# boqian333/E2ENet-Medical

Measured on AMD Instinct MI355X. Metric: voxels/sec (train step fwd+bwd+update), 128^3 patch 32ch density=0.2, higher is better.
Workload: dtype f32 (fp16x2 split products, f32 accumulate); 1 GPU; BraTS-shaped 4-modal 128^3 patches, shiftConvPP base 32, K=4, DSFF density 0.2, batch 2 per GPU, fwd+loss+bwd+clip+SGD+mask step, dense (parity) wgrad; parallelism=dp1

## Files before the change

e2enet_medical_amd/_lib.py:

```python
import ctypes as C
import os

_HERE = os.path.dirname(os.path.abspath(__file__))
LIB_PATH = os.environ.get("E2E_LIB_PATH") or os.path.join(_HERE, "csrc", "libe2e_hip.so")

KNOWN_ENV = frozenset({
    "E2E_CONV_MM", "E2E_MM_GRID", "E2E_MM_GEOM", "E2E_MM_PAIRQ", "E2E_CONV_DENSE", "E2E_CONV_SPARSE2", "E2E_CONV_PERSIST", "E2E_CONV_WGS",
    "E2E_CONV_KSPLIT", "E2E_WG_H2", "E2E_WG_BF3", "E2E_CT_BF3", "E2E_CT_H2",
    "E2E_CONV_DBG", "E2E_MM_STAMPS",
    "E2E_LIB_PATH", "E2E_STRICT_ENV", "E2E_DENSE_MIN_DENSITY", "E2E_MM_MIN_DENSITY", "E2E_WGRAD_STREAM", "E2E_LANES", "E2E_GRAPHS",
    "E2E_GRAPH_MAX_VOXELS", "E2E_PLAN_CACHE_GB", "E2E_SW_BLOCKING", "E2E_FORCE_DIST",
    "E2E_CPU_THREADS", "E2E_BENCH_DRY", "E2E_BENCH_DRY_FAIL_RANK", "E2E_BENCH_ALL_LAUNCHES",
})


def check_env(environ=None, strict=None):
    environ = os.environ if environ is None else environ
    unknown = sorted(k for k in environ if k.startswith("E2E_") and k not in KNOWN_ENV)
    if not unknown:
        return
    msg = ("unknown E2E_* environment variable(s) %s: not read by this build (known: %s)"
           % (", ".join(unknown), ", ".join(sorted(KNOWN_ENV))))
    if strict is None:
        strict = environ.get("E2E_STRICT_ENV") == "1"
# ... 77 lines not shown
    "e2e_conv133_mm_ws_bytes": (LL, [I, I, I, I, I, I, I, I, I]),
    "e2e_conv133_mm_pack": (I, [P, I, LL, P]),
    "e2e_conv133_input_ranges_ws_bytes": (LL, [I]),
    "e2e_conv133_input_ranges": (I, [P, I, P, P]),
    "e2e_absmax_word": (I, [P, LL, P, P]),
    "e2e_conv133_fwd_mm": (I, [P, I, P, P, P, P, P, P, I, I, I, I, I, P]),
    "e2e_conv133_dgrad_mm": (I, [P, P, P, P, P, I, I, I, I, I, I, P]),
    "e2e_conv133_dgrad_dense": (I, [P, P, P, P, I, I, I, I, I, I, P, LL, P]),
    "e2e_conv133_wgrad_ws_bytes": (LL, [I, I, I, I, I, I, I, I, I]),
    "e2e_conv133_wgrad": (I, [P, P, P, P, I, I, I, I, I, I, I, I, I, P, P, P]),
    "e2e_diag_split_gemm": (I, [P, P, P, I, I, P, P]),
    "e2e_diag_kernel_clock": (I, [I, P, P, I]),
    "e2e_in_stats_finalize": (I, [P, I, P, P, F, P, P, P, P, I, I, P]),
    "e2e_in_lrelu_bwd_ws_doubles": (LL, [I, I]),
    "e2e_in_lrelu_bwd": (I, [P, P, P, P, P, P, P, F, P, P, P, P, I, I, LL, P, I, P, P]),
    "e2e_convT_fwd": (I, [P, P, P, F, P, P, P, I, I, I, I, I, I, I, I, I, P, P, P]),
    "e2e_convT_dgrad": (I, [P, P, P, P, I, I, I, I, I, I, I, I, I, I, P, P, P, P]),
    "e2e_convT_wgrad_ws_bytes": (LL, [I, I, I, I, I, I, I, I, I]),
    "e2e_convT_wgrad": (I, [P, P, P, F, P, P, P, I, I, I, I, I, I, I, I, I, P, P, P, P]),
    "e2e_maxpool_fwd": (I, [P, P, P, F, P, I, I, I, I, I, I, I, I, P]),
    "e2e_maxpool_bwd_num_records": (I, [I, I, I, I, I, I]),
    "e2e_maxpool_bwd": (I, [P, P, P, F, P, P, I, I, I, I, I, I, I, I, I, P, P, P, P]),
    "e2e_head1x1_fwd": (I, [P, P, P, F, P, P, I, I, I, LL, P]),
    "e2e_head1x1_dgrad": (I, [P, P, P, I, I, I, I, LL, P]),
    "e2e_head1x1_wgrad_ws_bytes": (LL, [I, I, I, LL]),
    "e2e_head1x1_wgrad": (I, [P, P, P, F, P, P, P, I, I, I, LL, P]),
    "e2e_loss_ws_bytes": (LL, [I, I]),
    "e2e_dc_ce_reduce": (I, [P, P, P, I, I, LL, P]),
    "e2e_dc_ce_grad": (I, [P, P, P, F, I, F, P, P, I, I, LL, P]),
    "e2e_dc_ce_fold_batch": (I, [P, I, I, P]),
    "e2e_online_eval_counts": (I, [P, P, P, I, I, LL, P]),
    "e2e_dc_bce_reduce": (I, [P, P, P, P, I, I, LL, P]),
    "e2e_dc_bce_grad": (I, [P, P, P, P, F, I, F, P, P, I, I, LL, P]),
    "e2e_online_eval_regions": (I, [P, P, P, P, I, I, LL, P]),
    "e2e_seg_to_regions": (I, [P, P, P, I, I, LL, P]),
    "e2e_ds_target_gather": (I, [P, P, P, P, P, I, I, I, I, I, I, I, P]),
    "e2e_grad_sqnorm": (I, [P, I, P, P]),
# ... 59 lines not shown
    "e2e_pp_select_ws_bytes": (LL, [LL, I]),
    "e2e_pp_select_count": (I, [P, LL, P, I, P, P, P]),
    "e2e_pp_select_coords": (I, [P, I, I, I, P, I, P, P, P, P, P, P]),
    "e2e_fingerprint_sample_chunk": (I, []),
    "e2e_fingerprint_sample_ws_bytes": (LL, [LL]),
    "e2e_fingerprint_sample_count": (I, [P, LL, P, P, P]),
    "e2e_fingerprint_sample_gather": (I, [P, P, I, LL, I, P, LL, P, P]),
    "e2e_fingerprint_stats_max_ranks": (I, []),
    "e2e_fingerprint_stats_ws_bytes": (LL, []),
    "e2e_fingerprint_stats": (I, [P, LL, P, I, P, P, P]),
    "e2e_loader_crop_max_batch": (I, []),
    "e2e_loader_crop": (I, [P, I, I, I, I, I, P, P, I, F, F, P]),
}

_NO_STATUS = {"e2e_last_error", "e2e_abi_version", "e2e_last_kernel", "e2e_conv133_num_partials", "e2e_conv133_wgrad_ws_bytes", "e2e_conv133_dense_ws_bytes", "e2e_conv133_mm_ws_bytes", "e2e_conv133_sparse_eligible", "e2e_conv133_sparse_wpk_floats", "e2e_maxpool_bwd_num_records", "e2e_conv133_fwd_ws_bytes", "e2e_conv133_dgrad_ws_bytes",
              "e2e_convT_wgrad_ws_bytes", "e2e_conv133_input_ranges_ws_bytes", "e2e_in_lrelu_bwd_ws_doubles", "e2e_head1x1_wgrad_ws_bytes", "e2e_loss_ws_bytes", "e2e_aug_stats_ws_bytes",
              "e2e_surface_max_line", "e2e_surface_distances_ws_bytes", "e2e_cc_ws_bytes", "e2e_pp_nonzero_ws_bytes", "e2e_pp_label_hist_bins",
              "e2e_pp_minmax_ws_bytes", "e2e_pp_norm_ws_bytes", "e2e_pp_select_chunk", "e2e_pp_select_max_classes", "e2e_pp_select_ws_bytes",
              "e2e_fingerprint_sample_chunk", "e2e_fingerprint_sample_ws_bytes", "e2e_fingerprint_stats_max_ranks",
              "e2e_fingerprint_stats_ws_bytes", "e2e_eval_census_max_slots", "e2e_eval_census_chunk", "e2e_eval_census_workgroups",
              "e2e_loader_crop_max_batch"}


class E2EError(RuntimeError):
    pass


class _Lib:
    def __init__(self, path):
        if not os.path.exists(path):
            raise ImportError(
# ... 12 lines not shown

    def _checked(self, name, fn):
        last_error = self._dll.e2e_last_error

        def call(*a):
            rc = fn(*a)
            if rc != 0:
                raise E2EError("%s failed (%d): %s" % (name, rc, (last_error() or b"").decode()))
        call.__name__ = name
        return call


_lib = None


ABI_VERSION = 24


def lib() -> _Lib:
    global _lib
    if _lib is None:
        import torch
        check_env()
        handle = _Lib(LIB_PATH)
        got = handle.abi_version()
        if got != ABI_VERSION:
            raise ImportError("%s reports ABI version %d, this package needs %d: rebuild with `make -C %s`"
                              % (LIB_PATH, got, ABI_VERSION, os.path.dirname(LIB_PATH)))
        _lib = handle
    return _lib
```

e2enet_medical_amd/csrc/api.hip:

```cpp
#include "e2e_common.h"
#include <cstring>

namespace e2e {
static thread_local char g_err[512] = "";
void set_error(const char* fmt, ...) {
  va_list ap;
  va_start(ap, fmt);
  vsnprintf(g_err, sizeof(g_err), fmt, ap);
  va_end(ap);
}
static thread_local char g_kernel[160] = "";
void note_kernel(const char* fmt, ...) {
  va_list ap;
  va_start(ap, fmt);
  vsnprintf(g_kernel, sizeof(g_kernel), fmt, ap);
  va_end(ap);
}
}

extern "C" const char* e2e_last_error(void) { return e2e::g_err; }
extern "C" const char* e2e_last_kernel(void) { return e2e::g_kernel; }
extern "C" int e2e_abi_version(void) { return 24; }

extern "C" int e2e_diag_kernel_clock(int family, double* mhz, double* busy_ms, int reset) {
  E2E_REQUIRE(mhz != nullptr && (family == 0 || family == 1), "diag_kernel_clock: family 0 (conv133_mm) or 1 (conv133_wgrad v5)");
  if (hipDeviceSynchronize() != hipSuccess) return e2e::check_launch("diag_kernel_clock");
  unsigned long long v[2] = {0, 0};
  if (family == 0) e2e::mm_clock_read(v, reset != 0); else e2e::wgrad_clock_read(v, reset != 0);
  *mhz = v[1] ? 100.0 * (double)v[0] / (double)v[1] : 0.0;
  if (busy_ms) *busy_ms = (double)v[1] / 1e5;
  return e2e::check_launch("diag_kernel_clock");
}
```

e2enet_medical_amd/csrc/e2e_common.h:

```cpp
#pragma once
#include <hip/hip_runtime.h>
#include <cstdio>
#include <cstdarg>
#include "e2e_hip.h"

typedef const float __attribute__((address_space(1)))* gfloat_p;

namespace e2e {

void set_error(const char* fmt, ...);
void note_kernel(const char* fmt, ...);

void mm_clock_read(unsigned long long out[2], bool reset);
void wgrad_clock_read(unsigned long long out[2], bool reset);

inline int check_launch(const char* what) {
  hipError_t e = hipGetLastError();
  if (e != hipSuccess) {
    set_error("%s: %s", what, hipGetErrorString(e));
    return E2E_ERR_LAUNCH;
  }
  return E2E_OK;
}

// ... 75 lines not shown
  const e2e_in_chan_t* chans;
  const float* dy;
  float* slab;
  int B, Cin, Cout, Di, Hi, Wi, Do, sd;
  int tiles_x, tiles_y, tiles_per_n, tiles_per_chunk;
  int segs;
  int cblocks;
  int geom;
  int h2;
  const unsigned* dy_absmax;
  const unsigned* x_absmax;
};
int launch_wgrad_bf3(const WgBf3Params& p, int nchunks, int pairs, hipStream_t st);
int reduce_slabs(const float* slab, float* dw, long long numel, int nslabs, hipStream_t st);

inline int split_tiles(long long total, int pairs, int target_wgs, int min_tiles, int* tiles_per_chunk) {
  long long want = target_wgs / (pairs > 0 ? pairs : 1);
  if (want < 1) want = 1;
  long long tpc = cdivll(total, want);
  if (tpc < min_tiles) tpc = min_tiles;
  if (tpc > total) tpc = total;
  *tiles_per_chunk = (int)tpc;
  return (int)cdivll(total, tpc);
}
inline int split_tiles_per_item(int tiles_per_n, int B, int pairs, int target_wgs, int min_tiles, int* tiles_per_chunk, int* segs) {
  long long want = target_wgs / (pairs > 0 ? pairs : 1);
  if (want < B) want = B;
  int tpc = cdiv(tiles_per_n, (int)(want / B));
  if (tpc < min_tiles) tpc = min_tiles;
  if (tpc > tiles_per_n) tpc = tiles_per_n;
// ... 7 lines not shown
```

e2enet_medical_amd/csrc/instnorm.hip:

```cpp
#include "e2e_common.h"
#include "e2e_split.h"

namespace {

struct Stat {
  double n, mean, m2;
};
__device__ __forceinline__ Stat combine(const Stat a, const Stat b) {
  if (b.n == 0.0) return a;
  if (a.n == 0.0) return b;
  Stat r;
  r.n = a.n + b.n;
  const double delta = b.mean - a.mean;
  r.mean = a.mean + delta * (b.n / r.n);
  r.m2 = a.m2 + b.m2 + delta * delta * (a.n * b.n / r.n);
  return r;
}

__global__ __launch_bounds__(256) void in_finalize_kernel(const double* __restrict__ part, int np,
                                                          const float* __restrict__ gamma,
                                                          const float* __restrict__ beta, float eps,
                                                          float* __restrict__ scale, float* __restrict__ shift,
                                                          float* __restrict__ mean_out, float* __restrict__ rstd_out,
                                                          int C) {
// ... 95 lines not shown
  __syncthreads();
  if (threadIdx.x == 0) {
    double* r = sums + ((long long)nc * gridDim.x + blockIdx.x) * 2;
    r[0] = sh[0][0] + sh[0][1] + sh[0][2] + sh[0][3];
    r[1] = sh[1][0] + sh[1][1] + sh[1][2] + sh[1][3];
  }
}

__global__ __launch_bounds__(256) void in_bwd_apply_kernel(float* __restrict__ dz, const float* __restrict__ y,
                                                           const float* __restrict__ mean,
                                                           const float* __restrict__ rstd,
                                                           const float* __restrict__ scale,
                                                           const float* __restrict__ shift,
                                                           const float* __restrict__ gamma, float slope,
                                                           double* __restrict__ sums, const double* __restrict__ rec, int nrec,
                                                           int B, int C, long long spatial, unsigned* __restrict__ absmax,
                                                           double* __restrict__ rec3) {
  const int nc = blockIdx.y;
  const int c = nc % C;
  const float mu = mean[nc], rs = rstd[nc], g = gamma[c], sca = scale[nc], shf = shift[nc];
  __shared__ double s12[2];
  if (rec != nullptr) {
    if (threadIdx.x < 64) {
      const double* r = rec + (long long)nc * nrec * 2;
      double a = 0.0, b = 0.0;
      for (int i = threadIdx.x; i < nrec; i += 64) { a += r[2 * i]; b += r[2 * i + 1]; }
      a = e2e::wave_sum_d(a);
      b = e2e::wave_sum_d(b);
      if (threadIdx.x == 0) {
        s12[0] = a; s12[1] = b;
        if (blockIdx.x == 0) { sums[(long long)nc * 3] = a; sums[(long long)nc * 3 + 1] = b; }
      }
    }
  } else if (threadIdx.x == 0) {
// ... 122 lines not shown

}

extern "C" int e2e_in_stats_finalize(const double* part, int np, const float* gamma, const float* beta, float eps,
                                     float* scale, float* shift, float* mean, float* rstd, int B, int C,
                                     void* stream) {
  E2E_REQUIRE(part && gamma && beta && scale && shift && mean && rstd, "in_stats_finalize: null pointer");
  E2E_REQUIRE(np > 0 && B > 0 && C > 0, "in_stats_finalize: bad dims");
  hipLaunchKernelGGL(in_finalize_kernel, dim3(B * C), dim3(256), 0, (hipStream_t)stream, part, np, gamma, beta, eps,
                     scale, shift, mean, rstd, C);
  return e2e::check_launch("in_finalize_kernel");
}

extern "C" long long e2e_in_lrelu_bwd_ws_doubles(int B, int C) { return (long long)B * C * (3 + 3 * 256) + 2; }

extern "C" int e2e_in_lrelu_bwd(float* dz_dy, const float* y, const float* mean, const float* rstd, const float* scale,
                                const float* shift, const float* gamma, float slope, float* dgamma, float* dbeta,
                                float* dbias, float* sums, int B, int C, long long spatial, const double* tile_sums, int np,
                                unsigned* dy_absmax, void* stream) {
  E2E_REQUIRE(dz_dy && y && mean && rstd && scale && shift && gamma && dgamma && dbeta && sums, "in_lrelu_bwd: null pointer");
  E2E_REQUIRE(B > 0 && C > 0 && spatial > 0, "in_lrelu_bwd: bad dims");
  hipStream_t st = (hipStream_t)stream;
  double* ds = reinterpret_cast<double*>(sums);
  double* recs = ds + (long long)B * C * 3;
  double* rec3 = recs + (long long)B * C * 256 * 2;
  long long blocks = e2e::cdivll(spatial, 256 * 4 * 4);
  if (blocks > 256) blocks = 256;
  if (blocks < 1) blocks = 1;
  dim3 grid((unsigned)blocks, B * C);
  if (tile_sums == nullptr) {
    hipLaunchKernelGGL(in_bwd_reduce_kernel, grid, dim3(256), 0, st, dz_dy, y, mean, rstd, scale, shift, slope, recs, C,
                       spatial, dy_absmax, ds);
    hipLaunchKernelGGL(in_bwd_apply_kernel, grid, dim3(256), 0, st, dz_dy, y, mean, rstd, scale, shift, gamma, slope, ds,
                       (const double*)recs, (int)blocks, B, C, spatial, dy_absmax, rec3);
  } else {
    E2E_REQUIRE(np > 0, "in_lrelu_bwd: tile_sums without a record count");
    hipLaunchKernelGGL(in_bwd_tile_sums_kernel, dim3(B * C), dim3(64), 0, st, tile_sums, ds, np, dy_absmax);
    hipLaunchKernelGGL(in_bwd_apply_kernel, grid, dim3(256), 0, st, dz_dy, y, mean, rstd, scale, shift, gamma, slope, ds,
                       (const double*)nullptr, 0, B, C, spatial, dy_absmax, rec3);
  }
  hipLaunchKernelGGL(in_bwd_params_kernel, dim3(C), dim3(64), 0, st, (const double*)ds, (const double*)rec3, (int)blocks,
                     dgamma, dbeta, dbias, B, C);
  return e2e::check_launch("in_lrelu_bwd");
}
```

e2enet_medical_amd/csrc/pool_head.hip:

```cpp
#include "e2e_common.h"

namespace {

__global__ __launch_bounds__(256) void maxpool_fwd_kernel(const float* __restrict__ x, const float* __restrict__ scale,
                                                          const float* __restrict__ shift, float slope,
                                                          float* __restrict__ y, int D, int H, int W, int kd, int kh, int kw,
                                                          int Do, int Ho, int Wo) {
  const int nc = blockIdx.y;
  const long long ospatial = (long long)Do * Ho * Wo;
  const long long oi = (long long)blockIdx.x * 256 + threadIdx.x;
  if (oi >= ospatial) return;
  const int wo = (int)(oi % Wo);
  const long long r = oi / Wo;
  const int ho = (int)(r % Ho), dq = (int)(r / Ho);
  float a = 1.f, b = 0.f, sl = 1.f;
  if (scale) { a = scale[nc]; b = shift[nc]; sl = slope; }
  const float* xp = x + (long long)nc * D * H * W;
  float m = -INFINITY;
  for (int i = 0; i < kd; ++i)
    for (int j = 0; j < kh; ++j)
      for (int k = 0; k < kw; ++k) {
        const float v = e2e::in_act(xp[((long long)(dq * kd + i) * H + (ho * kh + j)) * W + (wo * kw + k)], a, b, sl);
        m = (v > m || v != v) ? v : m;
      }
// ... 401 lines not shown
    hipLaunchKernelGGL(maxpool_fwd_w2_kernel, grid2, dim3(256), 0, (hipStream_t)stream, x, scale, shift, slope, y, D, H, W, kd,
                       kh, Do, Ho, Wo);
    return e2e::check_launch("maxpool_fwd_w2_kernel");
  }
  dim3 grid((unsigned)e2e::cdivll((long long)Do * Ho * Wo, 256), B * C);
  hipLaunchKernelGGL(maxpool_fwd_kernel, grid, dim3(256), 0, (hipStream_t)stream, x, scale, shift, slope, y, D, H, W, kd, kh,
                     kw, Do, Ho, Wo);
  return e2e::check_launch("maxpool_fwd_kernel");
}

extern "C" int e2e_maxpool_bwd_num_records(int D, int H, int W, int kd, int kh, int kw) {
  if (kd < 1 || kh < 1 || kd > 2 || kh > 2 || kw != 2 || (W % 4) != 0 || D % kd || H % kh) return 0;
  return (int)e2e::cdivll((long long)(D / kd) * (H / kh) * (W / 4), 256);
}

extern "C" int e2e_maxpool_bwd(const float* x, const float* scale, const float* shift, float slope, const float* dy,
                               float* dx, int accumulate, int B, int C, int D, int H, int W, int kd, int kh, int kw,
                               const float* mean, const float* rstd, double* tile_sums, void* stream) {
  E2E_REQUIRE(x && dy && dx, "maxpool_bwd: null pointer");
  E2E_REQUIRE(kd >= 1 && kh >= 1 && kw >= 1 && D >= kd && H >= kh && W >= kw, "maxpool_bwd: bad dims");
  E2E_REQUIRE(tile_sums == nullptr || (mean && rstd && scale && e2e_maxpool_bwd_num_records(D, H, W, kd, kh, kw) > 0),
              "maxpool_bwd: fused InstanceNorm-backward sums need a normalised source and a shape of e2e_maxpool_bwd_num_records");
  hipStream_t st = (hipStream_t)stream;
  const int Do = D / kd, Ho = H / kh, Wo = W / kw;
  if (!accumulate && (D % kd || H % kh || W % kw)) {
    e2e::zero_async(dx, (size_t)B * C * D * H * W * sizeof(float), st);
  }
  if (kw == 2 && (W % 4) == 0 && kd <= 2 && kh <= 2) {
    dim3 grid2((unsigned)e2e::cdivll((long long)Do * Ho * (Wo / 2), 256), B * C);
    hipLaunchKernelGGL(maxpool_bwd_w2_kernel, grid2, dim3(256), 0, st, x, scale, shift, slope, dy, dx, accumulate, D, H, W, kd, kh,
                       Do, Ho, Wo, mean, rstd, tile_sums);
    return e2e::check_launch("maxpool_bwd_w2_kernel");
  }
  dim3 grid((unsigned)e2e::cdivll((long long)Do * Ho * Wo, 256), B * C);
  hipLaunchKernelGGL(maxpool_bwd_kernel, grid, dim3(256), 0, st, x, scale, shift, slope, dy, dx, accumulate, D, H, W, kd, kh,
                     kw, Do, Ho, Wo);
  return e2e::check_launch("maxpool_bwd_kernel");
}

#define DISPATCH_KB(K, ...)                                   \
  if ((K) <= 4) { constexpr int KB = 4; __VA_ARGS__; }        \
  else if ((K) <= 8) { constexpr int KB = 8; __VA_ARGS__; }   \
  else { constexpr int KB = 16; __VA_ARGS__; }

extern "C" int e2e_head1x1_fwd(const float* x, const float* scale, const float* shift, float slope, const float* w,
                               float* logits, int B, int C, int K, long long spatial, void* stream) {
// ... 60 lines not shown
```

e2enet_medical_amd/engine.py:

```python
import contextlib
import ctypes as C
import math
import os
from typing import Dict, List, Optional, Sequence, Tuple

import torch

import numpy as np

from ._lib import lib, InChan, OutChan, ParamEntry, SparsePackJob, InSumChan, MmPackJob, RangeSrc, RangeJob

LRELU_SLOPE = 0.01
IN_EPS = 1e-5
DENSE_MIN_DENSITY = float(os.environ.get("E2E_DENSE_MIN_DENSITY", "0.5"))
WGRAD_STREAM = os.environ.get("E2E_WGRAD_STREAM", "1") != "0"
WGRAD_STREAM_MAX_ELEMS = 40000000
WGRAD_LATE = True
LANES = os.environ.get("E2E_LANES", "1") != "0"
LANE_DIVS = None


def _lane_divs(voxels):
    if LANE_DIVS is not None:
        return LANE_DIVS
# ... 126 lines not shown
        for s in sources:
            assert s.shape[0] == b and s.shape[2:] == sources[0].shape[2:], "concat sources must agree spatially"
        self.cin = sum(s.shape[1] for s in sources)
        self.cout = cout
        self.in_dims = (di, hi, wi)
        sd, sh, sw = self.stride
        self.out_dims = ((di - 1) // sd + 1, (hi - 1) // sh + 1, (wi - 1) // sw + 1)
        self.out = Act(prefix, (b, cout) + self.out_dims, True, eng.device)
        self.out.producer = self
        self.dy_absmax = torch.zeros(1, dtype=torch.int32, device=eng.device)
        self.x_absmax = torch.zeros(1, dtype=torch.int32, device=eng.device)
        self.w_absmax = torch.zeros(1, dtype=torch.int32, device=eng.device)
        self.wpk_fwd = self.wpk_bwd = None
        self.own_sums = None
        self.own_np = 0
        self.np = lib().conv133_num_partials(*self.out_dims, sh, sw)
        self.part = torch.empty(b * cout * self.np * 3, dtype=torch.float64, device=eng.device)
        self.w_name = prefix + ".conv.weight"
        self.live = None
        self.live_t = None
        self.density = 1.0
        shifts = shift_amounts(self.cin, getattr(getattr(eng, 'cfg', None), 'shift_size', 5))
        structs = []
        c = 0
        for s in sources:
            cs = s.shape[1]
            plane = s.spatial
            for k in range(cs):
                structs.append(InChan(s.data.data_ptr() + 4 * k * plane,
                                      (s.scale.data_ptr() + 4 * k) if s.normed else None,
# ... 187 lines not shown
        L.in_stats_finalize(self.part.data_ptr(), self.np, p[self.prefix + ".instnorm.weight"].data_ptr(),
                            p[self.prefix + ".instnorm.bias"].data_ptr(), IN_EPS, self.out.scale.data_ptr(),
                            self.out.shift.data_ptr(), self.out.mean.data_ptr(), self.out.rstd.data_ptr(), b,
                            self.cout, _stream())

    def backward(self):
        e = self.eng
        p, g = e.params, e.grads
        o = self.out
        b = o.shape[0]
        di, hi, wi = self.in_dims
        sd, sh, sw = self.stride
        L = lib()
        ready = o.sums_ready
        o.sums_ready = False
        L.in_lrelu_bwd(o.grad.data_ptr(), o.data.data_ptr(), o.mean.data_ptr(), o.rstd.data_ptr(), o.scale.data_ptr(), o.shift.data_ptr(),
                       p[self.prefix + ".instnorm.weight"].data_ptr(),
                       LRELU_SLOPE, g[self.prefix + ".instnorm.weight"].data_ptr(),
                       g[self.prefix + ".instnorm.bias"].data_ptr(), g[self.prefix + ".conv.bias"].data_ptr(),
                       e.in_sums.data_ptr(), b, self.cout, o.spatial, self.own_sums.data_ptr() if ready else None, self.own_np,
                       self.dy_absmax.data_ptr(), _stream())
        late = WGRAD_LATE and getattr(e, "_wg_active", None) is not None and o.data.numel() > WGRAD_STREAM_MAX_ELEMS
        if not late:
            self._wgrad(e, L, g, o, b, di, hi, wi, sd, sh, sw, o.data.numel())
        if self.do_dgrad:
            ws = getattr(e, "fwd_ws", None)
            if self.use_mm("b"):
                if not hasattr(e, "_refresh_weight_caches"):
                    self.pack_mm_standalone("b")
                L.conv133_dgrad_mm(o.grad.data_ptr(), self.dy_absmax.data_ptr(), self.wpk_bwd.data_ptr(), self.w_absmax.data_ptr(),
                                   self.outs.data_ptr(), b, self.cin, self.cout, di, hi, wi, _stream())
            elif self.use_dense():
                L.conv133_dgrad_dense(o.grad.data_ptr(), p[self.w_name].data_ptr(), _ptr(self.live_t), self.outs.data_ptr(), b, self.cin, self.cout,
                                      di, hi, wi, ws.data_ptr(), ws.numel() * 4, _stream())
            elif self.sp_bwd is not None:
                sp = self.sp_bwd
# ... 116 lines not shown

    def wgrad_ws_bytes(self):
        b, cin, d, h, w = self.src.shape
        return lib().convT_wgrad_ws_bytes(b, cin, self.cout, d, h, w, *self.kernel)


class PoolOp:

    def __init__(self, eng, name, src: Act, kernel):
        self.eng, self.src, self.kernel = eng, src, tuple(kernel)
        b, c, d, h, w = src.shape
        kd, kh, kw = self.kernel
        self.out = Act(name, (b, c, d // kd, h // kh, w // kw), False, eng.device)
        self.out.pool_of = src.producer if src.normed else None
        self.acc = 0

    def plan_backward(self):
        self.src.alloc_grad()
        self.acc = self.src.claim_grad_write(self)

    def forward(self):
        s = self.src
        b, c, d, h, w = s.shape
        lib().maxpool_fwd(s.data.data_ptr(), _ptr(s.scale), _ptr(s.shift), LRELU_SLOPE, self.out.data.data_ptr(),
                          b, c, d, h, w, *self.kernel, _stream())

    def backward(self):
        s = self.src
        b, c, d, h, w = s.shape
        fuse = FUSE_IN_SUMS >= 1 and s.normed and s.last_writer is self and s.producer is not None and s.producer.own_sums is not None
        lib().maxpool_bwd(s.data.data_ptr(), _ptr(s.scale), _ptr(s.shift), LRELU_SLOPE, self.out.grad.data_ptr(),
                          s.grad.data_ptr(), self.acc, b, c, d, h, w, *self.kernel,
                          s.mean.data_ptr() if fuse else None, s.rstd.data_ptr() if fuse else None,
                          s.producer.own_sums.data_ptr() if fuse else None, _stream())
        if fuse:
            s.sums_ready = True


class HeadOp:

    def __init__(self, eng, w_name, src: Act, num_classes):
        self.eng, self.w_name, self.src, self.k = eng, w_name, src, num_classes
# ... 344 lines not shown
            order.remove(i)
            order.insert(order.index(index[id(prod)]), i)
        return order

    def _plan_lanes_backward(self):
        last = {}
        self._deps_bwd = [None] * len(self.ops)
        for i in self._bwd_order:
            op = self.ops[i]
            touched = [op.out] + [a for a in self._reads(op) if a.grad is not None]
            self._deps_bwd[i] = sorted({last[id(a)] for a in touched
                                        if id(a) in last and self._lane_of[last[id(a)]] != self._lane_of[i]})
            for a in touched:
                last[id(a)] = i
        self._ev_bwd = self._events_for(self._deps_bwd)

    @staticmethod
    def _events_for(deps):
        return {j: None for d in deps for j in d}

    def _lanes_on(self):
        return LANES and any(self._lane_of) and not self._graph_ok() and not torch.cuda.is_current_stream_capturing()

    def _exec(self, order, deps, events, action, checkpoint=None):
        main = torch.cuda.current_stream()
        if not self._lanes_on():
            for i in order:
                action(self.ops[i])
                if checkpoint is not None:
                    checkpoint(self.ops[i], lambda st: st.wait_stream(main))
# ... 104 lines not shown
        self._in_sums = [torch.zeros(int(lib().in_lrelu_bwd_ws_doubles(self.batch, cmax)), dtype=torch.float64, device=self.device)
                         for _ in range(len(self.lane_divs) + 1)]
        for op in self.conv_ops.values():
            d_, h_, w_ = op.out_dims
            lw = op.out.last_writer
            op.own_sums, op.own_np = None, 0
            if isinstance(lw, PoolOp) and FUSE_IN_SUMS >= 1:
                op.own_np = int(lib().maxpool_bwd_num_records(d_, h_, w_, *lw.kernel))
            elif isinstance(lw, ConvOp) and FUSE_IN_SUMS >= 2 and lw.sparse_ok:
                op.own_np = d_ * ((h_ + 15) // 16) * ((w_ + 31) // 32)
            if op.own_np > 0:
                op.own_sums = torch.zeros(self.batch * op.cout * op.own_np * 2, dtype=torch.float64, device=self.device)
            if op.sp_bwd is not None:
                op.sp_bwd.table = None
        self._plan_lanes_backward()
        self._loss_buffers()
        self._backward_ready = True

    def backward(self, dlogits: Optional[Sequence[Optional[torch.Tensor]]] = None):
        self.prepare_backward()
        if dlogits is not None:
            for h, g in zip(self.heads, dlogits):
                if g is None:
                    h.out.grad.zero_()
                else:
                    h.out.grad.copy_(g)
        for op in self.conv_ops.values():
            op.out.sums_ready = False
        self._refresh_weight_caches("b")
        hook = self.grad_bucket_hook
# ... 146 lines not shown
```

include/e2e_hip.h:

```cpp
#ifndef E2E_HIP_H
#define E2E_HIP_H

#ifdef __cplusplus
extern "C" {
#endif

#define E2E_OK 0
#define E2E_ERR_ARG (-1)
#define E2E_ERR_LAUNCH (-2)
#define E2E_ERR_UNSUPPORTED (-3)

const char* e2e_last_error(void);
int e2e_abi_version(void);
const char* e2e_last_kernel(void);

typedef struct {
  const float* ptr;
  const float* scale;
  const float* shift;
  long long nstride;
  int ab_nstride;
  int dshift;
  float slope;
  int reserved;
// ... 101 lines not shown
int e2e_conv133_wgrad(const e2e_in_chan_t* chans, const float* dy, float* dw, void* ws, int B, int Cin,
                      int Cout, int Di, int Hi, int Wi, int sd, int sh, int sw, const unsigned* dy_absmax,
                      const unsigned* x_absmax, void* stream);

int e2e_diag_split_gemm(const float* A, const float* Bt, float* D, int K, int mode, const unsigned* absmax_b, void* stream);

int e2e_diag_kernel_clock(int family, double* mhz, double* busy_ms, int reset);

int e2e_in_stats_finalize(const double* part, int np, const float* gamma, const float* beta, float eps,
                          float* scale, float* shift, float* mean, float* rstd, int B, int C, void* stream);

long long e2e_in_lrelu_bwd_ws_doubles(int B, int C);
int e2e_in_lrelu_bwd(float* dz_dy, const float* y, const float* mean, const float* rstd, const float* scale, const float* shift,
                     const float* gamma, float slope, float* dgamma, float* dbeta, float* dbias, float* sums,
                     int B, int C, long long spatial, const double* tile_sums, int np, unsigned* dy_absmax, void* stream);

int e2e_convT_fwd(const float* x, const float* scale, const float* shift, float slope, const float* w,
                  const unsigned* live, float* y, int B, int Cin, int Cout, int D, int H, int W, int kd,
                  int kh, int kw, const unsigned* x_absmax, const unsigned* w_absmax, void* stream);
int e2e_convT_dgrad(const float* dy, const float* w, const unsigned* live_t, float* dx, int accumulate, int B,
                    int Cin, int Cout, int D, int H, int W, int kd, int kh, int kw, const unsigned* w_absmax,
                    const unsigned* dy_bound_a, const unsigned* dy_bound_b, void* stream);
long long e2e_convT_wgrad_ws_bytes(int B, int Cin, int Cout, int D, int H, int W, int kd, int kh, int kw);
int e2e_convT_wgrad(const float* x, const float* scale, const float* shift, float slope, const float* dy,
                    float* dw, void* ws, int B, int Cin, int Cout, int D, int H, int W, int kd, int kh, int kw,
                    const unsigned* x_absmax, const unsigned* dy_bound_a, const unsigned* dy_bound_b, void* stream);

int e2e_maxpool_fwd(const float* x, const float* scale, const float* shift, float slope, float* y, int B, int C,
                    int D, int H, int W, int kd, int kh, int kw, void* stream);
int e2e_maxpool_bwd_num_records(int D, int H, int W, int kd, int kh, int kw);
int e2e_maxpool_bwd(const float* x, const float* scale, const float* shift, float slope, const float* dy,
                    float* dx, int accumulate, int B, int C, int D, int H, int W, int kd, int kh, int kw,
                    const float* mean, const float* rstd, double* tile_sums, void* stream);

int e2e_head1x1_fwd(const float* x, const float* scale, const float* shift, float slope, const float* w,
                    float* logits, int B, int C, int K, long long spatial, void* stream);
int e2e_head1x1_dgrad(const float* dlogits, const float* w, float* dx, int accumulate, int B, int C, int K,
                      long long spatial, void* stream);
long long e2e_head1x1_wgrad_ws_bytes(int B, int C, int K, long long spatial);
int e2e_head1x1_wgrad(const float* x, const float* scale, const float* shift, float slope,
                      const float* dlogits, float* dw, void* ws, int B, int C, int K, long long spatial,
                      void* stream);

long long e2e_loss_ws_bytes(int B, int K);
int e2e_dc_ce_reduce(const float* logits, const float* target, void* acc, int B, int K, long long spatial,
                     void* stream);
int e2e_dc_ce_grad(const float* logits, const float* target, const void* acc, float weight, int batch_dice,
                   float smooth, float* dlogits, float* loss_out, int B, int K, long long spatial, void* stream);
// ... 163 lines not shown
```

Baseline: 126.7 million voxels/s.

## Fold maxpool backward into instnorm-lrelu backward with optional cache-sized instance slices

```diff
diff --git a/e2enet_medical_amd/_lib.py b/e2enet_medical_amd/_lib.py
--- a/e2enet_medical_amd/_lib.py
+++ b/e2enet_medical_amd/_lib.py
@@ -6,7 +6,7 @@
 
 KNOWN_ENV = frozenset({
     "E2E_CONV_MM", "E2E_MM_GRID", "E2E_MM_GEOM", "E2E_MM_PAIRQ", "E2E_CONV_DENSE", "E2E_CONV_SPARSE2", "E2E_CONV_PERSIST", "E2E_CONV_WGS",
-    "E2E_CONV_KSPLIT", "E2E_WG_H2", "E2E_WG_BF3", "E2E_CT_BF3", "E2E_CT_H2",
+    "E2E_CONV_KSPLIT", "E2E_WG_H2", "E2E_WG_BF3", "E2E_CT_BF3", "E2E_CT_H2", "E2E_K7_SLICE_MB",
     "E2E_CONV_DBG", "E2E_MM_STAMPS",
     "E2E_LIB_PATH", "E2E_STRICT_ENV", "E2E_DENSE_MIN_DENSITY", "E2E_MM_MIN_DENSITY", "E2E_WGRAD_STREAM", "E2E_LANES", "E2E_GRAPHS",
     "E2E_GRAPH_MAX_VOXELS", "E2E_PLAN_CACHE_GB", "E2E_SW_BLOCKING", "E2E_FORCE_DIST",
@@ -115,6 +115,9 @@
     "e2e_in_stats_finalize": (I, [P, I, P, P, F, P, P, P, P, I, I, P]),
     "e2e_in_lrelu_bwd_ws_doubles": (LL, [I, I]),
     "e2e_in_lrelu_bwd": (I, [P, P, P, P, P, P, P, F, P, P, P, P, I, I, LL, P, I, P, P]),
+    "e2e_k7_slice_plan": (I, [LL, LL, LL, P, P, I]),
+    "e2e_k7_slice_bytes": (LL, []),
+    "e2e_set_k7_slice_bytes": (I, [LL]),
     "e2e_convT_fwd": (I, [P, P, P, F, P, P, P, I, I, I, I, I, I, I, I, I, P, P, P]),
     "e2e_convT_dgrad": (I, [P, P, P, P, I, I, I, I, I, I, I, I, I, I, P, P, P, P]),
     "e2e_convT_wgrad_ws_bytes": (LL, [I, I, I, I, I, I, I, I, I]),
@@ -122,6 +125,7 @@
     "e2e_maxpool_fwd": (I, [P, P, P, F, P, I, I, I, I, I, I, I, I, P]),
     "e2e_maxpool_bwd_num_records": (I, [I, I, I, I, I, I]),
     "e2e_maxpool_bwd": (I, [P, P, P, F, P, P, I, I, I, I, I, I, I, I, I, P, P, P, P]),
+    "e2e_maxpool_bwd_in_lrelu_bwd": (I, [P, I, I, I, I, I, I, I, P, P, P, P, P, P, P, P, F, P, P, P, P, I, I, P, P]),
     "e2e_head1x1_fwd": (I, [P, P, P, F, P, P, I, I, I, LL, P]),
     "e2e_head1x1_dgrad": (I, [P, P, P, I, I, I, I, LL, P]),
     "e2e_head1x1_wgrad_ws_bytes": (LL, [I, I, I, LL]),
@@ -211,7 +215,7 @@
 }
 
 _NO_STATUS = {"e2e_last_error", "e2e_abi_version", "e2e_last_kernel", "e2e_conv133_num_partials", "e2e_conv133_wgrad_ws_bytes", "e2e_conv133_dense_ws_bytes", "e2e_conv133_mm_ws_bytes", "e2e_conv133_sparse_eligible", "e2e_conv133_sparse_wpk_floats", "e2e_maxpool_bwd_num_records", "e2e_conv133_fwd_ws_bytes", "e2e_conv133_dgrad_ws_bytes",
-              "e2e_convT_wgrad_ws_bytes", "e2e_conv133_input_ranges_ws_bytes", "e2e_in_lrelu_bwd_ws_doubles", "e2e_head1x1_wgrad_ws_bytes", "e2e_loss_ws_bytes", "e2e_aug_stats_ws_bytes",
+              "e2e_convT_wgrad_ws_bytes", "e2e_conv133_input_ranges_ws_bytes", "e2e_in_lrelu_bwd_ws_doubles", "e2e_k7_slice_plan", "e2e_k7_slice_bytes", "e2e_head1x1_wgrad_ws_bytes", "e2e_loss_ws_bytes", "e2e_aug_stats_ws_bytes",
               "e2e_surface_max_line", "e2e_surface_distances_ws_bytes", "e2e_cc_ws_bytes", "e2e_pp_nonzero_ws_bytes", "e2e_pp_label_hist_bins",
               "e2e_pp_minmax_ws_bytes", "e2e_pp_norm_ws_bytes", "e2e_pp_select_chunk", "e2e_pp_select_max_classes", "e2e_pp_select_ws_bytes",
               "e2e_fingerprint_sample_chunk", "e2e_fingerprint_sample_ws_bytes", "e2e_fingerprint_stats_max_ranks",
@@ -254,7 +258,7 @@
 _lib = None
 
 
-ABI_VERSION = 24
+ABI_VERSION = 25
 
 
 def lib() -> _Lib:
diff --git a/e2enet_medical_amd/csrc/api.hip b/e2enet_medical_amd/csrc/api.hip
--- a/e2enet_medical_amd/csrc/api.hip
+++ b/e2enet_medical_amd/csrc/api.hip
@@ -20,7 +20,7 @@
 
 extern "C" const char* e2e_last_error(void) { return e2e::g_err; }
 extern "C" const char* e2e_last_kernel(void) { return e2e::g_kernel; }
-extern "C" int e2e_abi_version(void) { return 24; }
+extern "C" int e2e_abi_version(void) { return 25; }
 
 extern "C" int e2e_diag_kernel_clock(int family, double* mhz, double* busy_ms, int reset) {
   E2E_REQUIRE(mhz != nullptr && (family == 0 || family == 1), "diag_kernel_clock: family 0 (conv133_mm) or 1 (conv133_wgrad v5)");
diff --git a/e2enet_medical_amd/csrc/e2e_common.h b/e2enet_medical_amd/csrc/e2e_common.h
--- a/e2enet_medical_amd/csrc/e2e_common.h
+++ b/e2enet_medical_amd/csrc/e2e_common.h
@@ -113,6 +113,18 @@
 int launch_wgrad_bf3(const WgBf3Params& p, int nchunks, int pairs, hipStream_t st);
 int reduce_slabs(const float* slab, float* dw, long long numel, int nslabs, hipStream_t st);
 
+void launch_maxpool_bwd_w2(const float* x, const float* scale, const float* shift, float slope, const float* dy, float* dx,
+                           int accumulate, int instances, int D, int H, int W, int kd, int kh, const float* mean, const float* rstd,
+                           double* part, hipStream_t st);
+
+inline long long k7_slice_instances(long long instances, long long spatial, long long slice_bytes) {
+  if (slice_bytes <= 0 || spatial <= 0) return instances > 0 ? instances : 1;
+  long long per = slice_bytes / (8 * spatial);
+  if (per < 1) per = 1;
+  if (per > instances) per = instances > 0 ? instances : 1;
+  return per;
+}
+
 inline int split_tiles(long long total, int pairs, int target_wgs, int min_tiles, int* tiles_per_chunk) {
   long long want = target_wgs / (pairs > 0 ? pairs : 1);
   if (want < 1) want = 1;
diff --git a/e2enet_medical_amd/csrc/instnorm.hip b/e2enet_medical_amd/csrc/instnorm.hip
--- a/e2enet_medical_amd/csrc/instnorm.hip
+++ b/e2enet_medical_amd/csrc/instnorm.hip
@@ -1,5 +1,7 @@
 #include "e2e_common.h"
 #include "e2e_split.h"
+#include <atomic>
+#include <cstdlib>
 
 namespace {
 
@@ -133,10 +135,10 @@
                                                            const float* __restrict__ shift,
                                                            const float* __restrict__ gamma, float slope,
                                                            double* __restrict__ sums, const double* __restrict__ rec, int nrec,
-                                                           int B, int C, long long spatial, unsigned* __restrict__ absmax,
+                                                           int nc0, int C, long long spatial, unsigned* __restrict__ absmax,
                                                            double* __restrict__ rec3) {
   const int nc = blockIdx.y;
-  const int c = nc % C;
+  const int c = (nc0 + nc) % C;
   const float mu = mean[nc], rs = rstd[nc], g = gamma[c], sca = scale[nc], shf = shift[nc];
   __shared__ double s12[2];
   if (rec != nullptr) {
@@ -289,32 +291,117 @@
 
 extern "C" long long e2e_in_lrelu_bwd_ws_doubles(int B, int C) { return (long long)B * C * (3 + 3 * 256) + 2; }
 
+
+#ifndef K7_SLICE_ASCENDING
+#define K7_SLICE_ASCENDING 0
+#endif
+#ifndef K7_SLICE_DEFAULT_MB
+#define K7_SLICE_DEFAULT_MB 0
+#endif
+static std::atomic<long long> g_k7_slice_bytes{-1};
+
+extern "C" long long e2e_k7_slice_bytes(void) {
+  long long v = g_k7_slice_bytes.load(std::memory_order_relaxed);
+  if (v < 0) {
+    const char* s = getenv("E2E_K7_SLICE_MB");
+    const long long mb = s ? atoll(s) : (long long)K7_SLICE_DEFAULT_MB;
+    v = mb > 0 ? mb << 20 : 0;
+    g_k7_slice_bytes.store(v, std::memory_order_relaxed);
+  }
+  return v;
+}
+
+extern "C" int e2e_set_k7_slice_bytes(long long bytes) {
+  E2E_REQUIRE(bytes >= 0, "set_k7_slice_bytes: negative size (0 turns the slices off)");
+  g_k7_slice_bytes.store(bytes, std::memory_order_relaxed);
+  return E2E_OK;
+}
+
+extern "C" int e2e_k7_slice_plan(long long instances, long long spatial, long long slice_bytes, int* first, int* count, int cap) {
+  if (instances < 1 || spatial < 1 || instances > 0x7fffffffLL) return 0;
+  const long long per = e2e::k7_slice_instances(instances, spatial, slice_bytes);
+  const long long n = e2e::cdivll(instances, per);
+  for (long long k = 0; k < n && k < cap; ++k) {
+    if (first) first[k] = (int)(k * per);
+    if (count) count[k] = (int)(instances - k * per < per ? instances - k * per : per);
+  }
+  return (int)n;
+}
+
+namespace {
+
+struct K7Pool {
+  const float* dy;
+  int accumulate, D, H, W, kd, kh;
+  double* records;
+};
+
+int k7_run(float* dz_dy, const float* y, const float* mean, const float* rstd, const float* scale, const float* shift,
+           const float* gamma, float slope, float* dgamma, float* dbeta, float* dbias, float* sums, int B, int C, long long spatial,
+           const double* tile_sums, int np, unsigned* dy_absmax, const K7Pool* pool, hipStream_t st) {
+  double* ds = reinterpret_cast<double*>(sums);
+  double* recs = ds + (long long)B * C * 3;
+  double* rec3 = recs + (long long)B * C * 256 * 2;
+  long long blocks = e2e::cdivll(spatial, 256 * 4 * 4);
+  if (blocks > 256) blocks = 256;
+  if (blocks < 1) blocks = 1;
+  const long long inst = (long long)B * C;
+  const long long per = e2e::k7_slice_instances(inst, spatial, e2e_k7_slice_bytes());
+  const long long nslices = e2e::cdivll(inst, per);
+  for (long long k = 0; k < nslices; ++k) {
+    const long long f = (K7_SLICE_ASCENDING ? k : nslices - 1 - k) * per;
+    const long long cnt = inst - f < per ? inst - f : per;
+    unsigned* am = k == 0 ? dy_absmax : nullptr;
+    float* dzs = dz_dy + f * spatial;
+    const float* ys = y + f * spatial;
+    dim3 grid((unsigned)blocks, (unsigned)cnt);
+    if (pool != nullptr) {
+      const long long ospatial = (long long)(pool->D / pool->kd) * (pool->H / pool->kh) * (pool->W / 2);
+      e2e::launch_maxpool_bwd_w2(ys, scale + f, shift + f, slope, pool->dy + f * ospatial, dzs, pool->accumulate, (int)cnt, pool->D,
+                                 pool->H, pool->W, pool->kd, pool->kh, mean + f, rstd + f, pool->records + f * np * 2, st);
+    }
+    if (tile_sums == nullptr) {
+      hipLaunchKernelGGL(in_bwd_reduce_kernel, grid, dim3(256), 0, st, dzs, ys, mean + f, rstd + f, scale + f, shift + f, slope,
+                         recs + f * blocks * 2, C, spatial, am, ds + f * 3);
+      hipLaunchKernelGGL(in_bwd_apply_kernel, grid, dim3(256), 0, st, dzs, ys, mean + f, rstd + f, scale + f, shift + f, gamma, slope,
+                         ds + f * 3, (const double*)(recs + f * blocks * 2), (int)blocks, (int)f, C, spatial, dy_absmax, rec3 + f * blocks);
+    } else {
+      hipLaunchKernelGGL(in_bwd_tile_sums_kernel, dim3((unsigned)cnt), dim3(64), 0, st, tile_sums + f * np * 2, ds + f * 3, np, am);
+      hipLaunchKernelGGL(in_bwd_apply_kernel, grid, dim3(256), 0, st, dzs, ys, mean + f, rstd + f, scale + f, shift + f, gamma, slope,
+                         ds + f * 3, (const double*)nullptr, 0, (int)f, C, spatial, dy_absmax, rec3 + f * blocks);
+    }
+  }
+  hipLaunchKernelGGL(in_bwd_params_kernel, dim3(C), dim3(64), 0, st, (const double*)ds, (const double*)rec3, (int)blocks,
+                     dgamma, dbeta, dbias, B, C);
+  return E2E_OK;
+}
+
+}
+
 extern "C" int e2e_in_lrelu_bwd(float* dz_dy, const float* y, const float* mean, const float* rstd, const float* scale,
                                 const float* shift, const float* gamma, float slope, float* dgamma, float* dbeta,
                                 float* dbias, float* sums, int B, int C, long long spatial, const double* tile_sums, int np,
                                 unsigned* dy_absmax, void* stream) {
   E2E_REQUIRE(dz_dy && y && mean && rstd && scale && shift && gamma && dgamma && dbeta && sums, "in_lrelu_bwd: null pointer");
   E2E_REQUIRE(B > 0 && C > 0 && spatial > 0, "in_lrelu_bwd: bad dims");
-  hipStream_t st = (hipStream_t)stream;
-  double* ds = reinterpret_cast<double*>(sums);
-  double* recs = ds + (long long)B * C * 3;
-  double* rec3 = recs + (long long)B * C * 256 * 2;
-  long long blocks = e2e::cdivll(spatial, 256 * 4 * 4);
-  if (blocks > 256) blocks = 256;
-  if (blocks < 1) blocks = 1;
-  dim3 grid((unsigned)blocks, B * C);
-  if (tile_sums == nullptr) {
-    hipLaunchKernelGGL(in_bwd_reduce_kernel, grid, dim3(256), 0, st, dz_dy, y, mean, rstd, scale, shift, slope, recs, C,
-                       spatial, dy_absmax, ds);
-    hipLaunchKernelGGL(in_bwd_apply_kernel, grid, dim3(256), 0, st, dz_dy, y, mean, rstd, scale, shift, gamma, slope, ds,
-                       (const double*)recs, (int)blocks, B, C, spatial, dy_absmax, rec3);
-  } else {
-    E2E_REQUIRE(np > 0, "in_lrelu_bwd: tile_sums without a record count");
-    hipLaunchKernelGGL(in_bwd_tile_sums_kernel, dim3(B * C), dim3(64), 0, st, tile_sums, ds, np, dy_absmax);
-    hipLaunchKernelGGL(in_bwd_apply_kernel, grid, dim3(256), 0, st, dz_dy, y, mean, rstd, scale, shift, gamma, slope, ds,
-                       (const double*)nullptr, 0, B, C, spatial, dy_absmax, rec3);
-  }
-  hipLaunchKernelGGL(in_bwd_params_kernel, dim3(C), dim3(64), 0, st, (const double*)ds, (const double*)rec3, (int)blocks,
-                     dgamma, dbeta, dbias, B, C);
+  E2E_REQUIRE(tile_sums == nullptr || np > 0, "in_lrelu_bwd: tile_sums without a record count");
+  k7_run(dz_dy, y, mean, rstd, scale, shift, gamma, slope, dgamma, dbeta, dbias, sums, B, C, spatial, tile_sums, np, dy_absmax,
+         nullptr, (hipStream_t)stream);
   return e2e::check_launch("in_lrelu_bwd");
 }
+
+extern "C" int e2e_maxpool_bwd_in_lrelu_bwd(const float* pool_dy, int accumulate, int D, int H, int W, int kd, int kh, int kw,
+                                            double* records, float* dz_dy, const float* y, const float* mean, const float* rstd,
+                                            const float* scale, const float* shift, const float* gamma, float slope, float* dgamma,
+                                            float* dbeta, float* dbias, float* sums, int B, int C, unsigned* dy_absmax,
+                                            void* stream) {
+  E2E_REQUIRE(pool_dy && records && dz_dy && y && mean && rstd && scale && shift && gamma && dgamma && dbeta && sums,
+              "maxpool_bwd_in_lrelu_bwd: null pointer");
+  E2E_REQUIRE(B > 0 && C > 0, "maxpool_bwd_in_lrelu_bwd: bad dims");
+  const int np = e2e_maxpool_bwd_num_records(D, H, W, kd, kh, kw);
+  E2E_REQUIRE(np > 0, "maxpool_bwd_in_lrelu_bwd: a shape of e2e_maxpool_bwd_num_records > 0 only (use the two calls)");
+  const K7Pool pool{pool_dy, accumulate, D, H, W, kd, kh, records};
+  k7_run(dz_dy, y, mean, rstd, scale, shift, gamma, slope, dgamma, dbeta, dbias, sums, B, C, (long long)D * H * W, records, np,
+         dy_absmax, &pool, (hipStream_t)stream);
+  return e2e::check_launch("maxpool_bwd_in_lrelu_bwd");
+}
diff --git a/e2enet_medical_amd/csrc/pool_head.hip b/e2enet_medical_amd/csrc/pool_head.hip
--- a/e2enet_medical_amd/csrc/pool_head.hip
+++ b/e2enet_medical_amd/csrc/pool_head.hip
@@ -439,6 +439,20 @@
   return (int)e2e::cdivll((long long)(D / kd) * (H / kh) * (W / 4), 256);
 }
 
+static void launch_w2(const float* x, const float* scale, const float* shift, float slope, const float* dy, float* dx, int accumulate,
+                      int instances, int D, int H, int W, int kd, int kh, const float* mean, const float* rstd, double* part,
+                      hipStream_t st) {
+  const int Do = D / kd, Ho = H / kh, Wo = W / 2;
+  dim3 grid2((unsigned)e2e::cdivll((long long)Do * Ho * (Wo / 2), 256), instances);
+  hipLaunchKernelGGL(maxpool_bwd_w2_kernel, grid2, dim3(256), 0, st, x, scale, shift, slope, dy, dx, accumulate, D, H, W, kd, kh,
+                     Do, Ho, Wo, mean, rstd, part);
+}
+void e2e::launch_maxpool_bwd_w2(const float* x, const float* scale, const float* shift, float slope, const float* dy, float* dx,
+                                int accumulate, int instances, int D, int H, int W, int kd, int kh, const float* mean,
+                                const float* rstd, double* part, hipStream_t st) {
+  launch_w2(x, scale, shift, slope, dy, dx, accumulate, instances, D, H, W, kd, kh, mean, rstd, part, st);
+}
+
 extern "C" int e2e_maxpool_bwd(const float* x, const float* scale, const float* shift, float slope, const float* dy,
                                float* dx, int accumulate, int B, int C, int D, int H, int W, int kd, int kh, int kw,
                                const float* mean, const float* rstd, double* tile_sums, void* stream) {
@@ -452,9 +466,7 @@
     e2e::zero_async(dx, (size_t)B * C * D * H * W * sizeof(float), st);
   }
   if (kw == 2 && (W % 4) == 0 && kd <= 2 && kh <= 2) {
-    dim3 grid2((unsigned)e2e::cdivll((long long)Do * Ho * (Wo / 2), 256), B * C);
-    hipLaunchKernelGGL(maxpool_bwd_w2_kernel, grid2, dim3(256), 0, st, x, scale, shift, slope, dy, dx, accumulate, D, H, W, kd, kh,
-                       Do, Ho, Wo, mean, rstd, tile_sums);
+    launch_w2(x, scale, shift, slope, dy, dx, accumulate, B * C, D, H, W, kd, kh, mean, rstd, tile_sums, st);
     return e2e::check_launch("maxpool_bwd_w2_kernel");
   }
   dim3 grid((unsigned)e2e::cdivll((long long)Do * Ho * Wo, 256), B * C);
diff --git a/e2enet_medical_amd/engine.py b/e2enet_medical_amd/engine.py
--- a/e2enet_medical_amd/engine.py
+++ b/e2enet_medical_amd/engine.py
@@ -164,6 +164,7 @@
         self.wpk_fwd = self.wpk_bwd = None
         self.own_sums = None
         self.own_np = 0
+        self.fold_pool = None
         self.np = lib().conv133_num_partials(*self.out_dims, sh, sw)
         self.part = torch.empty(b * cout * self.np * 3, dtype=torch.float64, device=eng.device)
         self.w_name = prefix + ".conv.weight"
@@ -381,12 +382,21 @@
         L = lib()
         ready = o.sums_ready
         o.sums_ready = False
-        L.in_lrelu_bwd(o.grad.data_ptr(), o.data.data_ptr(), o.mean.data_ptr(), o.rstd.data_ptr(), o.scale.data_ptr(), o.shift.data_ptr(),
-                       p[self.prefix + ".instnorm.weight"].data_ptr(),
-                       LRELU_SLOPE, g[self.prefix + ".instnorm.weight"].data_ptr(),
-                       g[self.prefix + ".instnorm.bias"].data_ptr(), g[self.prefix + ".conv.bias"].data_ptr(),
-                       e.in_sums.data_ptr(), b, self.cout, o.spatial, self.own_sums.data_ptr() if ready else None, self.own_np,
-                       self.dy_absmax.data_ptr(), _stream())
+        pool = self.fold_pool
+        if pool is not None:
+            L.maxpool_bwd_in_lrelu_bwd(pool.out.grad.data_ptr(), pool.acc, *self.out_dims, *pool.kernel, self.own_sums.data_ptr(),
+                                       o.grad.data_ptr(), o.data.data_ptr(), o.mean.data_ptr(), o.rstd.data_ptr(), o.scale.data_ptr(),
+                                       o.shift.data_ptr(), p[self.prefix + ".instnorm.weight"].data_ptr(), LRELU_SLOPE,
+                                       g[self.prefix + ".instnorm.weight"].data_ptr(), g[self.prefix + ".instnorm.bias"].data_ptr(),
+                                       g[self.prefix + ".conv.bias"].data_ptr(), e.in_sums.data_ptr(), b, self.cout,
+                                       self.dy_absmax.data_ptr(), _stream())
+        else:
+            L.in_lrelu_bwd(o.grad.data_ptr(), o.data.data_ptr(), o.mean.data_ptr(), o.rstd.data_ptr(), o.scale.data_ptr(), o.shift.data_ptr(),
+                           p[self.prefix + ".instnorm.weight"].data_ptr(),
+                           LRELU_SLOPE, g[self.prefix + ".instnorm.weight"].data_ptr(),
+                           g[self.prefix + ".instnorm.bias"].data_ptr(), g[self.prefix + ".conv.bias"].data_ptr(),
+                           e.in_sums.data_ptr(), b, self.cout, o.spatial, self.own_sums.data_ptr() if ready else None, self.own_np,
+                           self.dy_absmax.data_ptr(), _stream())
         late = WGRAD_LATE and getattr(e, "_wg_active", None) is not None and o.data.numel() > WGRAD_STREAM_MAX_ELEMS
         if not late:
             self._wgrad(e, L, g, o, b, di, hi, wi, sd, sh, sw, o.data.numel())
@@ -533,6 +543,7 @@
         self.out = Act(name, (b, c, d // kd, h // kh, w // kw), False, eng.device)
         self.out.pool_of = src.producer if src.normed else None
         self.acc = 0
+        self.folded = False
 
     def plan_backward(self):
         self.src.alloc_grad()
@@ -545,6 +556,8 @@
                           b, c, d, h, w, *self.kernel, _stream())
 
     def backward(self):
+        if self.folded:
+            return
         s = self.src
         b, c, d, h, w = s.shape
         fuse = FUSE_IN_SUMS >= 1 and s.normed and s.last_writer is self and s.producer is not None and s.producer.own_sums is not None
@@ -919,6 +932,20 @@
             for a in touched:
                 last[id(a)] = i
         self._ev_bwd = self._events_for(self._deps_bwd)
+
+    def _plan_pool_folds(self):
+        index = {id(op): i for i, op in enumerate(self.ops)}
+        for k, i in enumerate(self._bwd_order[:-1]):
+            op = self.ops[i]
+            if not isinstance(op, PoolOp):
+                continue
+            s = op.src
+            prod = s.producer if s.normed else None
+            j = self._bwd_order[k + 1]
+            op.folded = (FUSE_IN_SUMS >= 1 and prod is not None and s.last_writer is op and prod.own_sums is not None
+                         and index.get(id(prod)) == j and self._lane_of[i] == self._lane_of[j] and i not in self._ev_bwd)
+            if op.folded:
+                prod.fold_pool = op
 
     @staticmethod
     def _events_for(deps):
@@ -1053,6 +1080,7 @@
             if op.sp_bwd is not None:
                 op.sp_bwd.table = None
         self._plan_lanes_backward()
+        self._plan_pool_folds()
         self._loss_buffers()
         self._backward_ready = True
 
diff --git a/include/e2e_hip.h b/include/e2e_hip.h
--- a/include/e2e_hip.h
+++ b/include/e2e_hip.h
@@ -139,6 +139,9 @@
 int e2e_in_lrelu_bwd(float* dz_dy, const float* y, const float* mean, const float* rstd, const float* scale, const float* shift,
                      const float* gamma, float slope, float* dgamma, float* dbeta, float* dbias, float* sums,
                      int B, int C, long long spatial, const double* tile_sums, int np, unsigned* dy_absmax, void* stream);
+int e2e_k7_slice_plan(long long instances, long long spatial, long long slice_bytes, int* first, int* count, int cap);
+long long e2e_k7_slice_bytes(void);
+int e2e_set_k7_slice_bytes(long long bytes);
 
 int e2e_convT_fwd(const float* x, const float* scale, const float* shift, float slope, const float* w,
                   const unsigned* live, float* y, int B, int Cin, int Cout, int D, int H, int W, int kd,
@@ -157,6 +160,10 @@
 int e2e_maxpool_bwd(const float* x, const float* scale, const float* shift, float slope, const float* dy,
                     float* dx, int accumulate, int B, int C, int D, int H, int W, int kd, int kh, int kw,
                     const float* mean, const float* rstd, double* tile_sums, void* stream);
+int e2e_maxpool_bwd_in_lrelu_bwd(const float* pool_dy, int accumulate, int D, int H, int W, int kd, int kh, int kw, double* records,
+                                 float* dz_dy, const float* y, const float* mean, const float* rstd, const float* scale,
+                                 const float* shift, const float* gamma, float slope, float* dgamma, float* dbeta, float* dbias,
+                                 float* sums, int B, int C, unsigned* dy_absmax, void* stream);
 
 int e2e_head1x1_fwd(const float* x, const float* scale, const float* shift, float slope, const float* w,
                     float* logits, int B, int C, int K, long long spatial, void* stream);
```

After: 126.8 million voxels/s (median of 2 runs). About the same (+0.1%).
